# jgkellymit/GENIE-SMEM

Measured on AMD Instinct MI355X. Metric: query-bases/sec SMEM discovery, 100kb ref x 150bp reads; bit-exact SMEM set, higher is better.
Workload: dtype u8/int32 (2-bit packed bases, int32 SA rows; f64 only in the RMI predict)

## Files before the change

genie-smem_amd/csrc/kernels.hip:

```cpp
#include <hip/hip_runtime.h>

#include <algorithm>
#include <cstdio>
#include <cstdlib>
#include <mutex>
#include <string>
#include <unordered_map>

#include "genie_internal.h"

namespace genie {

namespace {

constexpr int kWave = 64;

__device__ __forceinline__ int rfl(int v) { return __builtin_amdgcn_readfirstlane(v); }
__device__ __forceinline__ void set_wave_priority(int i)
{
    switch (i & 3) {
    case 0: __builtin_amdgcn_s_setprio(0); break;
    case 1: __builtin_amdgcn_s_setprio(1); break;
    case 2: __builtin_amdgcn_s_setprio(2); break;
    default: __builtin_amdgcn_s_setprio(3); break;
// ... 446 lines not shown
#pragma unroll
    for (int off = 32; off > 0; off >>= 1) {
        const unsigned int lo = (unsigned)__shfl_xor((int)(unsigned)v, off, kWave);
        const unsigned int hi = (unsigned)__shfl_xor((int)(unsigned)(v >> 32), off, kWave);
        v += ((unsigned long long)hi << 32) | lo;
    }
    return v;
}

__device__ __forceinline__ unsigned long long wave_inclusive_scan64(unsigned long long v, int lane)
{
#pragma unroll
    for (int off = 1; off < kWave; off <<= 1) {
        const unsigned int lo = (unsigned)__shfl_up((int)(unsigned)v, off, kWave);
        const unsigned int hi = (unsigned)__shfl_up((int)(unsigned)(v >> 32), off, kWave);
        if (lane >= off) v += ((unsigned long long)hi << 32) | lo;
    }
    return v;
}

__global__ void __launch_bounds__(kScanBlock) compact_block_sums(const int32_t *__restrict__ counts, long long N, int cap,
                                                                 unsigned long long *__restrict__ block_sums)
{
    __shared__ unsigned long long wsum[kScanBlock / kWave];
    const long long i = (long long)blockIdx.x * kScanBlock + threadIdx.x;
    unsigned long long v = 0;
    if (i < N) { const int c = counts[i]; v = (unsigned long long)(c < 0 ? 0 : (c < cap ? c : cap)); }
    v = wave_sum64(v);
    if ((threadIdx.x & 63) == 0) wsum[threadIdx.x >> 6] = v;
    __syncthreads();
    if (threadIdx.x == 0) {
        unsigned long long s = 0;
        for (int w = 0; w < kScanBlock / kWave; w++) s += wsum[w];
        block_sums[blockIdx.x] = s;
    }
}

__global__ void __launch_bounds__(kScanBlock) scan_block_sums_kernel(unsigned long long *__restrict__ sums, long long nblocks)
{
    constexpr int kPer = 8;
    __shared__ unsigned long long wave_total[kScanBlock / kWave];
    __shared__ unsigned long long carry;
    const int lane = threadIdx.x & (kWave - 1), wave = threadIdx.x >> 6;
    if (threadIdx.x == 0) carry = 0;
    __syncthreads();
    for (long long base = 0; base < nblocks; base += (long long)kScanBlock * kPer) {
        const long long i0 = base + (long long)threadIdx.x * kPer;
        unsigned long long v[kPer], mine = 0;
#pragma unroll
        for (int e = 0; e < kPer; e++) {
            v[e] = i0 + e < nblocks ? sums[i0 + e] : 0ull;
            mine += v[e];
        }
        unsigned long long inc = mine;
#pragma unroll
        for (int off = 1; off < kWave; off <<= 1) {
            const unsigned int lo = (unsigned)__shfl_up((int)(unsigned)inc, off, kWave);
            const unsigned int hi = (unsigned)__shfl_up((int)(unsigned)(inc >> 32), off, kWave);
            if (lane >= off) inc += ((unsigned long long)hi << 32) | lo;
        }
        if (lane == kWave - 1) wave_total[wave] = inc;
        __syncthreads();
        unsigned long long before = carry, all = 0;
        for (int w = 0; w < kScanBlock / kWave; w++) {
            const unsigned long long t = wave_total[w];
            before += w < wave ? t : 0ull;
            all += t;
        }
        unsigned long long run = before + inc - mine;
#pragma unroll
        for (int e = 0; e < kPer; e++) {
            if (i0 + e < nblocks) sums[i0 + e] = run;
            run += v[e];
        }
        __syncthreads();
        if (threadIdx.x == 0) carry += all;
        __syncthreads();
    }
    if (threadIdx.x == 0) sums[nblocks] = carry;
}

__global__ void __launch_bounds__(kScanBlock) compact_scatter(const int32_t *__restrict__ counts,
                                                              const int4 *__restrict__ slots, long long N, int cap,
                                                              const unsigned long long *__restrict__ block_sums,
                                                              long long *__restrict__ offsets, int4 *__restrict__ out,
                                                              long long out_cap_rows)
{
    __shared__ unsigned long long wave_total[kScanBlock / kWave];
    const int lane = threadIdx.x & (kWave - 1), wave = threadIdx.x >> 6;
    const long long i = (long long)blockIdx.x * kScanBlock + threadIdx.x;
    unsigned long long v = 0;
    if (i < N) { const int c = counts[i]; v = (unsigned long long)(c < 0 ? 0 : (c < cap ? c : cap)); }
    const unsigned long long inc = wave_inclusive_scan64(v, lane);
    if (lane == kWave - 1) wave_total[wave] = inc;
    __syncthreads();
    unsigned long long base = block_sums[blockIdx.x] + inc - v;
    for (int w = 0; w < wave; w++) base += wave_total[w];
    if (i < N) {
        offsets[i] = (long long)base;
        if (i == N - 1) offsets[N] = (long long)(base + v);
        if (out) {
            const long long room = out_cap_rows - (long long)base;
            const unsigned int fit = room <= 0 ? 0u : (room < (long long)v ? (unsigned int)room : (unsigned int)v);
            for (unsigned int t = 0; t < fit; t++) out[base + t] = slots[i * (long long)cap + t];
        }
    }
}

std::mutex g_err_mu;
std::string g_err;

#define HIP_TRY(expr)                                                         \
    do {                                                                      \
        hipError_t e_ = (expr);                                               \
        if (e_ != hipSuccess) { set_hip_error(#expr, (int)e_); return GENIE_E_HIP; } \
    } while (0)

#define LAUNCH(kernel, grid, block, lds, stream, ...)                         \
    do {                                                                      \
        hipLaunchKernelGGL(kernel, grid, block, lds, stream, __VA_ARGS__);    \
        HIP_TRY(hipGetLastError());                                           \
    } while (0)

inline long long table_bytes(const genie_index *ix)
{
    return (long long)((ix->dev.flags & kFlagCompactTable) ? sizeof(MatchRec16) : sizeof(MatchRec)) * ix->dev.mtab_entries;
}

struct Geometry {
    int grid, block, lds;
    int grp;
    int wps;
    int wide;
    int max_len;
    int fwd_stride;
    int fwd_lds;
    int qp_recs;
    int qp_stride;
    int kj_row;
};

inline void shape_for(int max_len, Geometry *g)
{
    g->max_len = max_len;
    g->wide = max_len > 255;
    g->qp_recs = g->wide ? (max_len + 31) / 32 : ((max_len + 8 + 31) / 32 + 1 + 1) / 2;
    g->fwd_stride = g->wide ? ((max_len * 2) + 15) & ~15 : std::max(16, (max_len + 15) & ~15);
    int dw = std::max(1, (max_len + 3) / 4);
    if ((dw & 1) == 0) dw++;
    g->fwd_lds = dw * 4;
    g->kj_row = (std::max(max_len, 1) + 1 + 7) & ~7;
    g->qp_stride = g->wide ? g->qp_recs : g->qp_recs + kPairHeadWords * 8 / 16;
}

int plan_find_smems(const genie_index *ix, int mode, int max_len, long long N, Geometry *g)
{
    (void)mode;
    const int lds_cap = 160 * 1024;
    shape_for(max_len, g);
    const int cus = ix->num_cus > 0 ? ix->num_cus : 256;
    const int wpb = 8;
    long long per_block;
    if (g->wide) {
        g->grp = 1;
        g->lds = wpb * mt_long_wave_bytes(max_len, g->qp_recs) + 16;
        per_block = wpb;
    } else {
        const int ml = std::max(max_len, 1);
        const int grp = ix->opt_group_positions > 0 ? ix->opt_group_positions / ml : kMtTarget / ml;
        g->grp = std::max(1, std::min(std::min(kMtMaxG, kWave / mt_pack_dwords(ml) * 4), grp));
        g->lds = wpb * mt_wave_bytes(g->grp, ml, g->qp_recs, g->fwd_stride) + 16 + mt_quad_table_bytes(g->grp, ml);
        per_block = (long long)wpb * g->grp;
    }
    if (g->lds > lds_cap) return GENIE_E_TOO_LONG;
    g->block = wpb * kWave;
    g->wps = !g->wide && table_bytes(ix) > kTableFitsL2 ? 4 : ((ix->dev.flags & kFlagCompactTable) ? 6 : 8);
    int bpc = std::min(lds_cap / g->lds, 4 * g->wps / wpb);
    if (ix->opt_search_blocks_per_cu > 0) bpc = std::min(bpc, ix->opt_search_blocks_per_cu);
    if (bpc < 1) bpc = 1;
    long long gr = (long long)cus * bpc;
    const long long need = (N + per_block - 1) / per_block;
    if (gr > need) gr = need;
    if (gr < 1) gr = 1;
    g->grid = (int)gr;
    return GENIE_OK;
}

struct Workspace {
    uint8_t *fwd;
    RefRec *qp;
    int32_t *status;
    uint8_t *kj;
    int32_t *counts;
    uint8_t *scan_tmp;
    int32_t *vlens;
};

inline int64_t ws_align(int64_t x) { return (x + 255) & ~(int64_t)255; }

struct Carver {
    uint8_t *base;
    int64_t at = 0;
    template <class T> void take(T *&piece, int64_t bytes)
    {
        piece = base ? reinterpret_cast<T *>(base + at) : nullptr;
        at += ws_align(bytes);
    }
};

inline int64_t block_sums_bytes(int64_t N) { return (N / 16 + 3) * 8; }

inline int64_t workspace_layout(uint8_t *base, int64_t N, const Geometry &g, Workspace *ws, int64_t vlens_n = 0)
{
    Carver c{base};
    c.take(ws->fwd, N * (int64_t)g.fwd_stride);
    c.take(ws->qp, N * (int64_t)g.qp_stride * 16);
    c.take(ws->status, N * 4);
    c.take(ws->kj, N * (int64_t)g.kj_row * (g.wide ? 4 : 2));
    c.take(ws->counts, N * 4);
    c.take(ws->scan_tmp, block_sums_bytes(N));
    c.take(ws->vlens, vlens_n * 4);
    return c.at + 256;
}

inline int carve_workspace(void *d_ws, int64_t ws_bytes, int64_t N, const Geometry &g, Workspace *ws, int64_t vlens_n = 0)
{
    if (!d_ws || ws_bytes < workspace_layout(static_cast<uint8_t *>(d_ws), N, g, ws, vlens_n) || (reinterpret_cast<uintptr_t>(d_ws) & 255) != 0)
        return GENIE_E_CAPACITY;
    return GENIE_OK;
}

constexpr long long kLongTwoLaneReads = 32768;

struct FindRequest : FindBatch {
    int32_t *counts = nullptr, *slots = nullptr;
    int32_t cap = 0;
    int64_t *offsets = nullptr;
    int32_t *rows = nullptr;
    int64_t cap_rows = 0;
    bool packed = false;
    int row_bytes = 8;
    uint8_t *counts8 = nullptr, *status8 = nullptr;
    int64_t *escapes = nullptr;
    int64_t cap_escapes = 0;
    bool both = false;

    explicit FindRequest(const FindBatch &b) : FindBatch(b) {}
};

constexpr int kLdsBytes = 160 * 1024;
std::mutex g_lds_mu;
std::unordered_map<const void *, int> g_lds_limit;

template <class Kernel>
int allow_large_lds(Kernel k)
{
    const void *fn = reinterpret_cast<const void *>(k);
    int limit;
    {
        std::lock_guard<std::mutex> lk(g_lds_mu);
        auto it = g_lds_limit.find(fn);
        if (it == g_lds_limit.end()) {
            hipFuncAttributes attr;
            HIP_TRY(hipFuncGetAttributes(&attr, fn));
            it = g_lds_limit.emplace(fn, kLdsBytes - (int)attr.sharedSizeBytes).first;
        }
        limit = it->second;
    }
    HIP_TRY(hipFuncSetAttribute(fn, hipFuncAttributeMaxDynamicSharedMemorySize, limit));
    return GENIE_OK;
}

template <class Kernel, class... Args>
int launch_match_table(Kernel km, const Geometry &g, hipStream_t s, Args... args)
{
    if (int rc = allow_large_lds(km)) return rc;
    LAUNCH(km, dim3(g.grid), dim3(g.block), g.lds, s, args...);
    return GENIE_OK;
}

template <int MODE, bool WIDE>
int launch_pipeline(const genie_index *ix, const Geometry &g, const FindRequest &r, const Workspace &ws, hipStream_t s)
{
    int32_t *st = r.status ? r.status : ws.status;
    int32_t *cnt = r.counts ? r.counts : ws.counts;
    const bool c16 = (ix->dev.flags & kFlagCompactTable) != 0;
    const long long mtab_bytes = table_bytes(ix);
    const int cus = ix->num_cus > 0 ? ix->num_cus : 256;
    const int max_len = std::max(g.max_len, 1);
    const int long_flags = ix->opt_search_all | ix->opt_scheduling << 16, flags = long_flags | ix->opt_debug << 8;
    if (ix->ev_search_begin) HIP_TRY(hipEventRecord((hipEvent_t)ix->ev_search_begin, s));
    int rc;
    if (WIDE && r.both)
        rc = launch_match_table(c16 ? match_table_long_both_kernel<true> : match_table_long_both_kernel<false>, g, s, ix->dev,
                                (int)MODE, r.reads, r.lens, (long long)r.N, r.stride, r.fixed_len, reinterpret_cast<uint8_t *>(ws.fwd),
                                g.fwd_stride, ws.qp, g.qp_recs, st, max_len, mtab_bytes, long_flags, cus, ws.vlens);
    else if (WIDE)
        rc = launch_match_table(c16 ? match_table_long_kernel<true> : match_table_long_kernel<false>, g, s, ix->dev, (int)MODE,
                                r.reads, r.lens, (long long)r.N, r.stride, r.fixed_len, reinterpret_cast<uint8_t *>(ws.fwd),
                                g.fwd_stride, ws.qp, g.qp_recs, st, max_len, mtab_bytes, long_flags, cus);
    else if (r.both)
        rc = launch_match_table(c16 ? (g.wps == 4 ? match_table_both_kernel<4, true> : match_table_both_kernel<6, true>)
                                    : (g.wps == 4 ? match_table_both_kernel<4, false> : match_table_both_kernel<8, false>),
                                g, s, ix->dev, (int)MODE, r.reads, r.lens, (long long)r.N, r.stride, r.fixed_len,
                                reinterpret_cast<uint8_t *>(ws.fwd), g.fwd_stride, ws.qp, g.qp_recs, g.qp_stride, st, g.grp,
                                max_len, mtab_bytes, flags, cus, ws.vlens);
// ... 421 lines not shown
```

genie-smem_amd/csrc/match_table_body.inc:

```
    static_assert(!(PK && RC), "both strands of 2-bit packed reads are not built");
    typedef uint32_t __attribute__((aligned(1))) u32_unaligned;
    extern __shared__ __align__(16) uint8_t smem[];
    const int lane = threadIdx.x & (kWave - 1);
    const int wave = rfl((int)(threadIdx.x >> 6));
    const int waves_per_block = blockDim.x >> 6;
    const int dbg = (flags >> 8) & 63;
    const int sched = flags >> 16;
    const bool look_up_all = (flags & 1) != 0;
    const int FS = fwd_stride;
    const int K = ix.K;
    const int P2 = ix.P2;
    const int DW = mt_short_row_dwords(max_len, qp_recs);
    const int DWp = mt_pack_dwords(max_len);
    const int QL = mt_quads(max_len);
    const int nquads = grp * QL;
    const __amdgpu_buffer_rsrc_t mtab =
        __builtin_amdgcn_make_buffer_rsrc(const_cast<MatchRec *>(ix.mtab), 0, (int)mtab_bytes, 0x00020000);
    const __amdgpu_buffer_rsrc_t ov =
        __builtin_amdgcn_make_buffer_rsrc(const_cast<MatchOv16 *>(ix.ov), 0, ix.ov_entries * (int)sizeof(MatchOv16), 0x00020000);

    uint8_t *wb = smem + wave * mt_wave_bytes(grp, max_len, qp_recs, FS);
    uint32_t *Dp = reinterpret_cast<uint32_t *>(wb);
    int *Ls = reinterpret_cast<int *>(wb + mt_r16(grp * DW * 4));
    uint8_t *fwL = reinterpret_cast<uint8_t *>(Ls) + 64;
    uint16_t *sl = reinterpret_cast<uint16_t *>(fwL + mt_r16(grp * FS));
    uint16_t *qa = reinterpret_cast<uint16_t *>(reinterpret_cast<uint8_t *>(sl) + mt_r16(grp * max_len * 2));
    uint16_t *qb = qa + grp * mt_quads(max_len);
    for (int i = lane; i < grp * DW; i += kWave) Dp[i] = 0;
    const uint8_t *reads_end = reads + (RC ? N >> 1 : N) * (long long)stride;

    const int pu = (int)(((uint32_t)lane * (uint32_t)(65536 / DWp + 1)) >> 16);
    const int pj = lane - pu * DWp;

    uint32_t *next_group = reinterpret_cast<uint32_t *>(smem + waves_per_block * mt_wave_bytes(grp, max_len, qp_recs, FS));
    const long long groups = (N + grp - 1) / grp;
    const long long share = (groups + gridDim.x - 1) / gridDim.x;
    const long long g_begin = (long long)blockIdx.x * share;
    const long long g_end = g_begin + share < groups ? g_begin + share : groups;
    const bool handed_out = !(sched & 1), rotate = !(sched & 2);
    if (threadIdx.x == 0) *next_group = (uint32_t)waves_per_block;
    uint2 *qtab = reinterpret_cast<uint2 *>(next_group + 4);
    for (int t = threadIdx.x; t < (nquads + 191) / 192 * 192; t += blockDim.x) {
        const int tq = t < nquads ? t : 0;
        const int u = tq / QL, a = 4 * (tq - u * QL);
        const uint32_t o = 2u * (uint32_t)a + 1u;
        qtab[t] = make_uint2((uint32_t)u << 28 | (uint32_t)(u * FS + a) << 16 | (uint32_t)a,
                             ((uint32_t)(u * DW) + (o >> 5)) << 8 | (32u - (o & 31u)));
    }
    __syncthreads();
    long long gi = handed_out ? g_begin + wave : (long long)blockIdx.x * waves_per_block + wave;
    const long long g_stop = handed_out ? g_end : groups;
    const int round_of_block = (int)(blockIdx.x / (uint32_t)cus);
    const bool touch_ahead = !(sched & 8);
    for (int it = 0; gi < g_stop; it++) {
        const long long r = gi * grp;
        if (rotate) set_wave_priority(it + round_of_block);
        long long gi_next;
        if (handed_out) {
            uint32_t nx = 0;
            if (lane == 0) nx = atomicAdd(next_group, 1u);
            gi_next = g_begin + (long long)(uint32_t)rfl((int)nx);
        } else {
            gi_next = gi + (long long)gridDim.x * waves_per_block;
        }
        if (touch_ahead && stride > 0 && gi_next < g_stop) {
            const long long rn = gi_next * grp;
            const long long rows = N - rn < (long long)grp ? N - rn : (long long)grp;
            if (RC) scalar_touch_lines(reads + (rn >> 1) * (long long)stride, (uint32_t)((((rn + rows - 1) >> 1) - (rn >> 1) + 1) * stride));
            else scalar_touch_lines(reads + rn * (long long)stride, (uint32_t)(rows * stride));
        }
        bool any_read = false;
        for (int u0 = 0; u0 < grp; u0 += kWave / DWp) {
            const int u = u0 + pu;
            const bool mine = pu < kWave / DWp && u < grp;
            int L = 0, st = GENIE_READ_OK;
            uint32_t d = 0;
            bool bad = false;
            if (mine && r + u < N) {
                const long long row = RC ? (r + u) >> 1 : r + u;
                const bool rev = RC && ((r + u) & 1);
                L = lens ? lens[row] : fixed_len;
                if (RC && lens && pj == 0) vlens[r + u] = L;
                if (L < 0 || L > max_len) { st = GENIE_READ_BAD_BASE; L = 0; }
                const int left = L - 16 * pj;
                if (PK) {
                    if (left > 0) {
                        d = __builtin_bswap32(*reinterpret_cast<const uint32_t *>(reads + (r + u) * (long long)stride + 4 * pj));
                        if (left < 16) d &= ~0u << (32 - 2 * left);
                    }
                }
                const uint8_t *src = reads + row * (long long)stride + 16 * pj;
                uint32_t v[4] = {0, 0, 0, 0};
                if (PK) {
                } else if (rev) {
                    const long long o = row * (long long)stride + L - 16 - 16 * pj;
                    if (left >= 16 || (left > 0 && o >= 0)) {
                        const nt_u4 q = *reinterpret_cast<const nt_u4_unaligned *>(reads + o);
                        v[0] = __builtin_bswap32(q.w); v[1] = __builtin_bswap32(q.z); v[2] = __builtin_bswap32(q.y); v[3] = __builtin_bswap32(q.x);
                        if (left < 16) {
#pragma unroll
                            for (int k = 0; k < 4; k++) {
                                const int nb = left - 4 * k;
                                v[k] = nb >= 4 ? v[k] : (nb <= 0 ? 0u : v[k] & ((1u << (8 * nb)) - 1u));
                            }
                        }
                    } else if (left > 0) {
                        const uint8_t *f = reads + row * (long long)stride;
                        for (int b = 0; b < left; b++) v[b >> 2] |= (uint32_t)f[left - 1 - b] << (8 * (b & 3));
                    }
                } else if (left >= 16 || (left > 0 && src + 16 <= reads_end)) {
                    const nt_u4 q = *reinterpret_cast<const nt_u4_unaligned *>(src);
                    v[0] = q.x; v[1] = q.y; v[2] = q.z; v[3] = q.w;
                    if (left < 16) {
#pragma unroll
                        for (int k = 0; k < 4; k++) {
                            const int nb = left - 4 * k;
                            v[k] = nb >= 4 ? v[k] : (nb <= 0 ? 0u : v[k] & ((1u << (8 * nb)) - 1u));
                        }
                    }
                } else if (left > 0) {
#pragma unroll
                    for (int k = 0; k < 4; k++) {
                        if (left >= 4 * k + 4) v[k] = *reinterpret_cast<const u32_unaligned *>(src + 4 * k);
                        else for (int b = 0; b < left - 4 * k; b++) v[k] |= (uint32_t)src[4 * k + b] << (8 * b);
                    }
                }
                if (!PK) {
                    bad = ((v[0] | v[1] | v[2] | v[3]) & 0xFCFCFCFCu) != 0;
                    d = (mt_pack4(v[0]) << 24) | (mt_pack4(v[1]) << 16) | (mt_pack4(v[2]) << 8) | mt_pack4(v[3]);
                    if (rev && left > 0) d ^= left >= 16 ? ~0u : ~0u << (32 - 2 * left);
                }
            }
            const uint32_t prev = (uint32_t)__builtin_amdgcn_update_dpp(0, (int)d, 0x138 , 0xf, 0xf, true);
            const unsigned long long badm = __ballot(bad);
            bool ok = false;
            if (mine) {
                Dp[u * DW + pj] = __builtin_amdgcn_alignbit(prev, d, 1);
                if (pj == 0) {
                    const unsigned long long mine_bits = ((1ull << DWp) - 1ull) << (pu * DWp);
                    if (st == GENIE_READ_OK && (badm & mine_bits)) st = GENIE_READ_BAD_BASE;
                    if (st == GENIE_READ_OK && mode != GENIE_MODE_BWA && L < K) st = GENIE_READ_TOO_SHORT;
                    if (r + u < N) status[r + u] = st;
                    ok = st == GENIE_READ_OK && L > 0;
                    Ls[u] = ok ? L : 0;
                }
            }
            any_read |= __any(ok);
        }
        wave_lds_fence();
        if (any_read) {
            for (int t0 = 0; t0 < ((dbg & 8) ? 0 : grp * qp_recs); t0 += kWave) {
                const int t = t0 + lane;
                const int u = t / qp_recs, i = t - u * qp_recs;
                if (t < grp * qp_recs && Ls[u] > 0) {
                    const uint32_t *q = Dp + u * DW + 4 * i;
                    const uint32_t q0 = q[0], q1 = q[1], q2 = q[2], q3 = q[3], q4 = q[4];
                    uint4 rec;
                    rec.y = __builtin_amdgcn_alignbit(q0, q1, 31);
                    rec.x = __builtin_amdgcn_alignbit(q1, q2, 31);
                    rec.w = __builtin_amdgcn_alignbit(q2, q3, 31);
                    rec.z = __builtin_amdgcn_alignbit(q3, q4, 31);
                    store_nt(qp_out + (r + u) * (long long)qp_stride + i, rec);
                }
            }
            int nslow = 0;
#pragma nounroll
            for (int c0 = 0; c0 < ((dbg & 4) ? 0 : nquads); c0 += kMtNsp * kWave) {
                uint32_t ent[kMtNsp];
                MtProbe pr[kMtNsp];
#pragma unroll
                for (int s = 0; s < kMtNsp; s++) {
                    const int t0 = c0 + 64 * s + lane;
                    const uint2 q = qtab[t0];
                    int m = Ls[q.x >> 28] - (int)(q.x & 255u);
                    m = t0 < nquads && m > 0 ? m : 0;
                    ent[s] = q.x | ((uint32_t)m << 8);
                    const uint32_t *dq = Dp + (q.y >> 8);
                    const uint32_t sh = q.y & 255u;
                    const uint32_t d0 = dq[0], d1 = dq[1], d2 = dq[2];
                    pr[s] = mt_issue<C16>(mtab, __builtin_amdgcn_alignbit(d0, d1, sh), __builtin_amdgcn_alignbit(d1, d2, sh), P2);
                }
                mt_v4i rb[kMtNsp];
#pragma unroll
                for (int s = 0; s < kMtNsp; s++) rb[s] = mt_second<C16>(mtab, pr[s]);
#pragma unroll
                for (int s = 0; s < kMtNsp; s++) {
                    bool slow;
                    const int best0 = mt_eval<C16>(pr[s], rb[s], P2, slow);
                    const int a = (int)(ent[s] & 255u), m = (int)((ent[s] >> 8) & 255u);
                    const int best = best0 < m ? best0 : m;
                    if (m) fwL[(ent[s] >> 16) & 0xFFFu] = (uint8_t)(a + best);
                    slow = slow && m > best0;
                    const unsigned long long sb = __ballot(slow);
                    if (slow) sl[nslow + __popcll(sb & ((1ull << lane) - 1ull))] = (uint16_t)(((ent[s] >> 28) << 8) | (uint32_t)a);
                    nslow += __popcll(sb);
                }
            }
            wave_lds_fence();
#pragma nounroll
            for (int c0 = 0; c0 < ((dbg & 1) ? 0 : nslow); c0 += kWave) mt_slow<false, C16>(ix, mtab, ov, mode, lane, c0, nslow, sl, Dp, DW, Ls, fwL, FS);
            wave_lds_fence();
            nslow = 0;
            int nqa = 0, nqb = 0;
            const unsigned long long below = (1ull << lane) - 1ull;
#pragma nounroll
            for (int t0 = lane; t0 < ((dbg & 6) ? 0 : nquads) + lane; t0 += kWave) {
                const uint2 q = qtab[t0 < nquads ? t0 : 0];
                const int u = (int)(q.x >> 28), a = (int)(q.x & 255u);
                const int L = Ls[u];
                const int m = t0 < nquads && L > a ? L - a : 0;
                const uint32_t fo = (q.x >> 16) & 0xFFFu;
                const uint32_t v0 = fwL[fo];
                const bool has_right = m > 4;
                const uint32_t v4 = has_right ? fwL[fo + 4] : 0u;
                const bool need = m > 1 && (look_up_all || ((int)v0 != L && !(has_right && v4 == v0)));
                if (m && !need) *reinterpret_cast<uint32_t *>(fwL + fo) = v0 * 0x01010101u;
                const unsigned long long nb = __ballot(need);
                if (need) qa[nqa + __popcll(nb & below)] = (uint16_t)((uint32_t)u << 8 | (uint32_t)a);
                nqa += __popcll(nb);
            }
            wave_lds_fence();
#pragma nounroll
            for (int c0 = 0; c0 < nqa; c0 += kWave) {
                const bool valid = c0 + lane < nqa;
                const uint32_t it = qa[valid ? c0 + lane : 0];
                const int u = (int)(it >> 8), a = (int)(it & 255u);
                const int L = Ls[u], m = L - a;
                const int km = m > 2 ? 2 : 1;
                const uint32_t fo = __umul24((uint32_t)u, (uint32_t)FS) + (uint32_t)a;
                const uint32_t o = 2u * (uint32_t)(a + km) + 1u;
                const uint32_t *dq = Dp + __umul24((uint32_t)u, (uint32_t)DW) + (o >> 5);
                const uint32_t sh = 32u - (o & 31u);
                const uint32_t d0 = dq[0], d1 = dq[1], d2 = dq[2];
                const MtProbe pm = mt_issue<C16>(mtab, __builtin_amdgcn_alignbit(d0, d1, sh), __builtin_amdgcn_alignbit(d1, d2, sh), P2);
                const uint32_t v0 = fwL[fo];
                const bool has_right = m > 4;
                const uint32_t v4 = has_right ? fwL[fo + 4] : 0u;
                const mt_v4i rm = mt_second<C16>(mtab, pm);
                bool sm;
                const int bm = mt_eval<C16>(pm, rm, P2, sm);
                const int em = bm < m - km ? bm : m - km;
                sm = valid && sm && m - km > bm;
                const uint32_t vm = (uint32_t)(a + km + em);
                bool need1 = false, need3 = false;
                if (valid) {
                    if (km == 1) {
                        *reinterpret_cast<uint32_t *>(fwL + fo) = v0 | vm << 8;
                    } else {
                        need1 = look_up_all || sm || vm != v0;
                        need3 = m > 3 && (look_up_all || sm || !((has_right && vm == v4) || (int)vm == L));
                        *reinterpret_cast<uint32_t *>(fwL + fo) = v0 | v0 << 8 | vm << 16 | (m > 3 ? vm : 0u) << 24;
                    }
                }
                const unsigned long long sbm = __ballot(sm), b1 = __ballot(need1), b3 = __ballot(need3);
                if (sm) sl[nslow + __popcll(sbm & below)] = (uint16_t)(it + (uint32_t)km);
                nslow += __popcll(sbm);
                if (need1) qb[nqb + __popcll(b1 & below)] = (uint16_t)(it + 1u);
                nqb += __popcll(b1);
                if (need3) qb[nqb + __popcll(b3 & below)] = (uint16_t)(it + 3u);
                nqb += __popcll(b3);
            }
            wave_lds_fence();
#pragma nounroll
            for (int c0 = 0; c0 < nqb; c0 += kWave) {
                const bool valid = c0 + lane < nqb;
                const uint32_t it = qb[valid ? c0 + lane : 0];
                const int u = (int)(it >> 8), a = (int)(it & 255u);
                const int m = Ls[u] - a;
                const uint32_t o = 2u * (uint32_t)a + 1u;
                const uint32_t *dq = Dp + __umul24((uint32_t)u, (uint32_t)DW) + (o >> 5);
                const uint32_t sh = 32u - (o & 31u);
                const uint32_t d0 = dq[0], d1 = dq[1], d2 = dq[2];
                const MtProbe pn = mt_issue<C16>(mtab, __builtin_amdgcn_alignbit(d0, d1, sh), __builtin_amdgcn_alignbit(d1, d2, sh), P2);
                const mt_v4i rn = mt_second<C16>(mtab, pn);
                bool slow;
                const int b0 = mt_eval<C16>(pn, rn, P2, slow);
                const int e = b0 < m ? b0 : m;
                if (valid) fwL[__umul24((uint32_t)u, (uint32_t)FS) + (uint32_t)a] = (uint8_t)(a + e);
                slow = valid && slow && m > b0;
                const unsigned long long sb = __ballot(slow);
                if (slow) sl[nslow + __popcll(sb & below)] = (uint16_t)it;
                nslow += __popcll(sb);
            }
            wave_lds_fence();
#pragma nounroll
            for (int c0 = 0; c0 < ((dbg & 1) ? 0 : nslow); c0 += kWave) mt_slow<false, C16>(ix, mtab, ov, mode, lane, c0, nslow, sl, Dp, DW, Ls, fwL, FS);
            wave_lds_fence();
            const int nrows = N - r < (long long)grp ? (int)(N - r) : grp;
            uint4 *dst = reinterpret_cast<uint4 *>(fwd_out + r * (long long)FS);
            const uint4 *src = reinterpret_cast<const uint4 *>(fwL);
            for (int i = lane; i < ((dbg & 32) ? 0 : nrows * (FS >> 4)); i += kWave) store_nt(dst + i, src[i]);
        }
        wave_lds_fence();
        gi = gi_next;
    }
```

genie-smem_amd/csrc/match_table_kernel.inc:

```

constexpr int kMtNsp = 3;
constexpr int kMtMaxG = 16;
constexpr int kMtTarget = 768;


__host__ __device__ inline int mt_row_dwords(int max_len, int qp_recs)
{
    const int a = ((2 * (max_len + 8) + 1) >> 5) + 3, b = 2 * qp_recs + 3;
    return a > b ? a : b;
}
__host__ __device__ inline int mt_pack_dwords(int max_len) { return (max_len + 15) / 16 + 1; }
__host__ __device__ inline int mt_quads(int max_len) { return (max_len + 3) / 4; }
__host__ __device__ inline int mt_r16(int x) { return (x + 15) & ~15; }
__host__ __device__ inline int mt_quad_table_bytes(int grp, int max_len) { return (grp * mt_quads(max_len) + 191) / 192 * 192 * 8; }
__host__ __device__ inline int mt_short_row_dwords(int max_len, int chunks) { return mt_row_dwords(max_len, 2 * chunks - 1); }
__host__ __device__ inline int mt_wave_bytes(int grp, int max_len, int qp_recs, int fwd_stride)
{
    return mt_r16(grp * mt_short_row_dwords(max_len, qp_recs) * 4) + 64 + mt_r16(grp * fwd_stride) + mt_r16(grp * max_len * 2) +
           mt_r16(grp * mt_quads(max_len) * 6);
}

struct QBits {
    const uint32_t *p;
    __device__ __forceinline__ uint64_t win(int pos) const
    {
        const uint32_t o = 2u * (uint32_t)pos + 1u;
        const uint32_t *d = p + (o >> 5);
        const uint32_t s = 32u - (o & 31u);
        const uint32_t d0 = d[0], d1 = d[1], d2 = d[2];
        return ((uint64_t)__builtin_amdgcn_alignbit(d0, d1, s) << 32) | __builtin_amdgcn_alignbit(d1, d2, s);
    }
};

__device__ __forceinline__ uint32_t mt_pack4(uint32_t v) { return ((v << 6) | (v >> 4) | (v >> 14) | (v >> 24)) & 255u; }

struct MtProbe {
    uint32_t xk;
    int voff;
    mt_v4i ra;
};
template <bool C16>
__device__ __forceinline__ MtProbe mt_issue(const __amdgpu_buffer_rsrc_t mtab, uint32_t w1, uint32_t w2, int P2)
{
    MtProbe p;
    p.xk = __builtin_amdgcn_alignbit(w1, w2, 32 - 2 * P2);
    p.voff = (int)((w1 >> (32 - 2 * P2)) << (C16 ? 4 : 5));
    p.ra = __builtin_amdgcn_raw_buffer_load_b128(mtab, p.voff, 0, 0);
    return p;
}
template <bool C16>
__device__ __forceinline__ mt_v4i mt_second(const __amdgpu_buffer_rsrc_t mtab, const MtProbe &p)
{
    mt_v4i rb = mt_v4i{p.ra.z, p.ra.z, p.ra.z, p.ra.z};
    if (!C16 && ((uint32_t)p.ra.x >> 24) > 2u && p.xk > (uint32_t)p.ra.w) rb = __builtin_amdgcn_raw_buffer_load_b128(mtab, p.voff + 16, 0, 0);
    return rb;
}
typedef unsigned short mt_us2 __attribute__((ext_vector_type(2)));
__device__ __forceinline__ uint32_t mt_pk_min(uint32_t a, uint32_t b)
{
    return __builtin_bit_cast(uint32_t, __builtin_elementwise_min(__builtin_bit_cast(mt_us2, a), __builtin_bit_cast(mt_us2, b)));
}
__device__ __forceinline__ uint32_t mt_xmin16(const mt_v4i e, uint32_t xk16, bool more)
{
    const uint32_t xx = xk16 * 0x10001u;
    uint32_t d3 = (uint32_t)e.w ^ xx;
    d3 |= more ? 0xFFFF0000u : 0u;
    const uint32_t mm = mt_pk_min(mt_pk_min((uint32_t)e.y ^ xx, (uint32_t)e.z ^ xx), d3);
    return min(mm & 0xFFFFu, mm >> 16);
}
__device__ __forceinline__ int mt_lcp16(uint32_t x16) { return x16 ? (__clz((int)x16) - 16) >> 1 : 8; }
template <bool C16>
__device__ __forceinline__ int mt_eval(const MtProbe &p, const mt_v4i rb, int P2, bool &slow)
{
    if (C16) {
        const uint32_t w0 = (uint32_t)p.ra.x, cnt4 = (w0 >> 24) & 15u, nib = w0 >> 28;
        const bool wide = (nib & kM16Wide) && cnt4 >= 1u && cnt4 <= 3u;
        const bool rows_decide = cnt4 == kM16More || (cnt4 != 0 && !wide && (nib & kM16General));
        const uint32_t xx = wide ? p.xk : (p.xk >> 16) * 0x10001u;
        const uint32_t d1 = (uint32_t)p.ra.y ^ xx, d2 = (uint32_t)p.ra.z ^ xx, d3 = (uint32_t)p.ra.w ^ xx;
        const uint32_t mm = mt_pk_min(mt_pk_min(d1, d2), d3);
        const uint32_t xn = (min(mm & 0xFFFFu, mm >> 16) << 16) | 0xFFFFu;
        const uint32_t xw = min(min(d1, d2), d3);
        const int lcp = __clz((int)(wide ? xw : xn)) >> 1;
        slow = cnt4 != 0 && (rows_decide || lcp == (wide ? 16 : 8));
        return cnt4 == 0 ? (int)nib : (rows_decide ? P2 : P2 + lcp);
    }
    const uint32_t meta = (uint32_t)p.ra.x;
    uint32_t x = min(p.xk ^ (uint32_t)p.ra.z, p.xk ^ (uint32_t)p.ra.w);
    x = min(x, min(min(p.xk ^ (uint32_t)rb.x, p.xk ^ (uint32_t)rb.y), min(p.xk ^ (uint32_t)rb.z, p.xk ^ (uint32_t)rb.w)));
    const int lcp = __clz((int)x) >> 1;
    const int lm = (int)((meta >> 8) & 0x1Fu);
    slow = (meta & kMatchSlow) || lcp + lm == 16 + 0x1F;
    return (int)(meta & 0xFFu) + (lcp & lm);
}

struct MtQuad {
    uint32_t v1, v2, v3;
    bool s1, s2, s3;
};
template <bool C16>
__device__ __forceinline__ MtQuad mt_quad_interior(const __amdgpu_buffer_rsrc_t mtab, int P2, uint32_t d0, uint32_t d1, uint32_t d2,
                                                   uint32_t sh, int a, int m, int L, uint32_t v0, bool has_right, uint32_t v4,
                                                   bool look_up_all)
{
    MtQuad q{v0, 0u, 0u, false, false, false};
    const int km = m > 2 ? 2 : 1;
    const MtProbe pm = mt_issue<C16>(mtab, __builtin_amdgcn_alignbit(d0, d1, sh - 2 * km), __builtin_amdgcn_alignbit(d1, d2, sh - 2 * km), P2);
    const mt_v4i rm = mt_second<C16>(mtab, pm);
    bool sm;
    const int bm = mt_eval<C16>(pm, rm, P2, sm);
    const int em = bm < m - km ? bm : m - km;
    sm = sm && m - km > bm;
    const uint32_t vm = (uint32_t)(a + km + em);
    if (km == 1) {
        q.v1 = vm;
        q.s1 = sm;
        return q;
    }
    q.v2 = vm;
    q.s2 = sm;
    const bool need1 = look_up_all || sm || vm != v0;
    const bool need3 = m > 3 && (look_up_all || sm || !((has_right && vm == v4) || (int)vm == L));
    q.v1 = v0;
    q.v3 = m > 3 ? vm : 0u;
    if (need1 || need3) {
        const uint32_t s13 = need1 ? sh - 2 : sh - 6;
        const MtProbe pa = mt_issue<C16>(mtab, __builtin_amdgcn_alignbit(d0, d1, s13), __builtin_amdgcn_alignbit(d1, d2, s13), P2);
        MtProbe pb = pa;
        const bool both = need1 && need3;
        if (both) pb = mt_issue<C16>(mtab, __builtin_amdgcn_alignbit(d0, d1, sh - 6), __builtin_amdgcn_alignbit(d1, d2, sh - 6), P2);
        const mt_v4i ra = mt_second<C16>(mtab, pa);
        mt_v4i rb = ra;
        if (both) rb = mt_second<C16>(mtab, pb);
        bool sa, sb;
        const int ba = mt_eval<C16>(pa, ra, P2, sa), bb = mt_eval<C16>(pb, rb, P2, sb);
        const int ka = need1 ? 1 : 3;
        const int ea = ba < m - ka ? ba : m - ka, eb = bb < m - 3 ? bb : m - 3;
        sa = sa && m - ka > ba;
        sb = sb && m - 3 > bb;
        if (need1) { q.v1 = (uint32_t)(a + 1 + ea); q.s1 = sa; }
        else { q.v3 = (uint32_t)(a + 3 + ea); q.s3 = sa; }
        if (both) { q.v3 = (uint32_t)(a + 3 + eb); q.s3 = sb; }
    }
    return q;
}

template <bool LONG, bool C16, class QB = QBits, class FW = uint16_t>
__device__ __forceinline__ void mt_slow(const DevIndex &ix, const __amdgpu_buffer_rsrc_t mtab, const __amdgpu_buffer_rsrc_t ov, int mode, int lane, int c0,
                                        int count, const uint16_t *list, const uint32_t *Dp, int DW, const int *Ls,
                                        uint8_t *fwL, int FS, int L0 = 0, int wbase = 0, FW *fwW = nullptr)
{
    const int K = ix.K, P = ix.P, P2 = ix.P2;
    const int idx = c0 + lane;
    const bool on = idx < count;
    int u = 0, a = 0, m = 0, best = 0, chain = 0, cvoff = 0, nrows = 0;
    uint32_t mask = 0, lb = 0, c = 0, xmin = ~0u, xkq = 0;
    bool general = false;
    uint64_t w = 0, xq = 0;
    QB Q{reinterpret_cast<decltype(QB::p)>(Dp)};
    if (on) {
        const uint32_t e = (uint32_t)list[idx];
        if constexpr (LONG) {
            a = wbase + (int)e;
            m = L0 - a;
        } else {
            u = (int)(e >> 8);
            a = (int)(e & 255u);
            m = Ls[u] - a;
            Q.p = Dp + u * DW;
        }
        w = Q.win(a);
        xq = Q.win(a + P);
// ... 185 lines not shown
```

Baseline: 200.3 billion.

## Fuse quad-need scan into probe loop and defer plateau-dependent quads

The separate pass that re-read qtab and fwL to decide which quads need refinement is folded into the main probe loop, using per-quad slow-state bytes stored in a new LDS array. Quads whose outcome depends on an unresolved slow neighbour are placed on a deferred list and re-checked only after the slow path runs, so many skip the refinement probes. This removes one full LDS scan and a fence-separated slow pass before the scan, at the cost of extra LDS per wave, a second refinement trip, and more complex bookkeeping. A static_assert is added to keep three blocks per CU within LDS at 150 bases.

```diff
diff --git a/genie-smem_amd/csrc/kernels.hip b/genie-smem_amd/csrc/kernels.hip
--- a/genie-smem_amd/csrc/kernels.hip
+++ b/genie-smem_amd/csrc/kernels.hip
@@ -622,6 +622,9 @@
     g->kj_row = (std::max(max_len, 1) + 1 + 7) & ~7;
     g->qp_stride = g->wide ? g->qp_recs : g->qp_recs + kPairHeadWords * 8 / 16;
 }
+
+static_assert(3 * (8 * mt_wave_bytes(kMtTarget / 150, 150, 3, 160) + 16 + mt_quad_table_bytes(kMtTarget / 150, 150)) <= 160 * 1024,
+              "three blocks of the match-statistics kernel per CU no longer fit the LDS at 150 bases");
 
 int plan_find_smems(const genie_index *ix, int mode, int max_len, long long N, Geometry *g)
 {
diff --git a/genie-smem_amd/csrc/match_table_body.inc b/genie-smem_amd/csrc/match_table_body.inc
--- a/genie-smem_amd/csrc/match_table_body.inc
+++ b/genie-smem_amd/csrc/match_table_body.inc
@@ -26,6 +26,8 @@
     uint16_t *sl = reinterpret_cast<uint16_t *>(fwL + mt_r16(grp * FS));
     uint16_t *qa = reinterpret_cast<uint16_t *>(reinterpret_cast<uint8_t *>(sl) + mt_r16(grp * max_len * 2));
     uint16_t *qb = qa + grp * mt_quads(max_len);
+    uint16_t *qd = reinterpret_cast<uint16_t *>(reinterpret_cast<uint8_t *>(qa) + mt_r16(grp * mt_quads(max_len) * 6));
+    uint8_t *ss = reinterpret_cast<uint8_t *>(qd) + mt_r16(grp * mt_quads(max_len) * 2);
     for (int i = lane; i < grp * DW; i += kWave) Dp[i] = 0;
     const uint8_t *reads_end = reads + (RC ? N >> 1 : N) * (long long)stride;
 
@@ -163,7 +165,9 @@
                     store_nt(qp_out + (r + u) * (long long)qp_stride + i, rec);
                 }
             }
-            int nslow = 0;
+            int nslow = 0, nqa = 0, nqd = 0;
+            const unsigned long long below = (1ull << lane) - 1ull;
+            const bool list_on = !(dbg & 2);
 #pragma nounroll
             for (int c0 = 0; c0 < ((dbg & 4) ? 0 : nquads); c0 += kMtNsp * kWave) {
                 uint32_t ent[kMtNsp];
@@ -183,47 +187,60 @@
                 mt_v4i rb[kMtNsp];
 #pragma unroll
                 for (int s = 0; s < kMtNsp; s++) rb[s] = mt_second<C16>(mtab, pr[s]);
+                uint32_t vs[kMtNsp];
 #pragma unroll
                 for (int s = 0; s < kMtNsp; s++) {
                     bool slow;
                     const int best0 = mt_eval<C16>(pr[s], rb[s], P2, slow);
                     const int a = (int)(ent[s] & 255u), m = (int)((ent[s] >> 8) & 255u);
                     const int best = best0 < m ? best0 : m;
-                    if (m) fwL[(ent[s] >> 16) & 0xFFFu] = (uint8_t)(a + best);
                     slow = slow && m > best0;
+                    const bool plateau = C16 ? best0 != P2 : !((uint32_t)pr[s].ra.x & kMatchSlow);
+                    const uint32_t state = slow ? (plateau ? 2u : 1u) : 0u;
+                    vs[s] = (uint32_t)(a + best) | state << 8;
+                    if (m) {
+                        fwL[(ent[s] >> 16) & 0xFFFu] = (uint8_t)(a + best);
+                        ss[c0 + 64 * s + lane] = (uint8_t)state;
+                    }
                     const unsigned long long sb = __ballot(slow);
                     if (slow) sl[nslow + __popcll(sb & ((1ull << lane) - 1ull))] = (uint16_t)(((ent[s] >> 28) << 8) | (uint32_t)a);
                     nslow += __popcll(sb);
                 }
-            }
-            wave_lds_fence();
-#pragma nounroll
-            for (int c0 = 0; c0 < ((dbg & 1) ? 0 : nslow); c0 += kWave) mt_slow<false, C16>(ix, mtab, ov, mode, lane, c0, nslow, sl, Dp, DW, Ls, fwL, FS);
-            wave_lds_fence();
-            nslow = 0;
-            int nqa = 0, nqb = 0;
-            const unsigned long long below = (1ull << lane) - 1ull;
-#pragma nounroll
-            for (int t0 = lane; t0 < ((dbg & 6) ? 0 : nquads) + lane; t0 += kWave) {
-                const uint2 q = qtab[t0 < nquads ? t0 : 0];
-                const int u = (int)(q.x >> 28), a = (int)(q.x & 255u);
-                const int L = Ls[u];
-                const int m = t0 < nquads && L > a ? L - a : 0;
-                const uint32_t fo = (q.x >> 16) & 0xFFFu;
-                const uint32_t v0 = fwL[fo];
-                const bool has_right = m > 4;
-                const uint32_t v4 = has_right ? fwL[fo + 4] : 0u;
-                const bool need = m > 1 && (look_up_all || ((int)v0 != L && !(has_right && v4 == v0)));
-                if (m && !need) *reinterpret_cast<uint32_t *>(fwL + fo) = v0 * 0x01010101u;
-                const unsigned long long nb = __ballot(need);
-                if (need) qa[nqa + __popcll(nb & below)] = (uint16_t)((uint32_t)u << 8 | (uint32_t)a);
-                nqa += __popcll(nb);
-            }
-            wave_lds_fence();
+                wave_lds_fence();
+#pragma unroll
+                for (int s = 0; s < kMtNsp; s++) {
+                    const int a = (int)(ent[s] & 255u), m = (int)((ent[s] >> 8) & 255u);
+                    const int L = a + m;
+                    const uint32_t fo = (ent[s] >> 16) & 0xFFFu;
+                    const uint32_t v0 = vs[s] & 255u, s0 = vs[s] >> 8;
+                    const bool has_right = m > 4;
+                    const bool known = !(s == kMtNsp - 1 && lane == kWave - 1);
+                    const uint32_t v4 = has_right ? (known ? (uint32_t)fwL[fo + 4] : 256u) : 0u;
+                    const uint32_t s4 = has_right ? (known ? (uint32_t)ss[c0 + 64 * s + lane + 1] : 1u) : 0u;
+                    const bool x0 = s0 == 0u, x4 = s4 == 0u;
+                    const bool settled = x0 && ((int)v0 == L || (has_right && x4 && v4 == v0));
+                    const bool open = list_on && m > 1 && (look_up_all || !settled);
+                    const bool defer = open && !look_up_all && (x0 ? !x4 && v0 >= v4 : s0 == 2u);
+                    const bool need = open && !defer;
+                    if (list_on && m && !open) *reinterpret_cast<uint32_t *>(fwL + fo) = v0 * 0x01010101u;
+                    const unsigned long long nb = __ballot(need), db = __ballot(defer);
+                    const uint32_t item = (ent[s] >> 28) << 8 | (uint32_t)a;
+                    if (need) qa[nqa + __popcll(nb & below)] = (uint16_t)(item | (x0 ? 0u : 1u) | (x4 ? 0u : 2u));
+                    nqa += __popcll(nb);
+                    if (defer) qd[nqd + __popcll(db & below)] = (uint16_t)item;
+                    nqd += __popcll(db);
+                }
+            }
+            wave_lds_fence();
+            int nqb = 0;
+#pragma nounroll
+            for (int trip = 0;; trip++) {
 #pragma nounroll
             for (int c0 = 0; c0 < nqa; c0 += kWave) {
                 const bool valid = c0 + lane < nqa;
-                const uint32_t it = qa[valid ? c0 + lane : 0];
+                const uint32_t itf = qa[valid ? c0 + lane : 0];
+                const uint32_t it = itf & ~3u;
+                const bool f0 = (itf & 1u) != 0, f4 = (itf & 2u) != 0;
                 const int u = (int)(it >> 8), a = (int)(it & 255u);
                 const int L = Ls[u], m = L - a;
                 const int km = m > 2 ? 2 : 1;
@@ -247,8 +264,8 @@
                     if (km == 1) {
                         *reinterpret_cast<uint32_t *>(fwL + fo) = v0 | vm << 8;
                     } else {
-                        need1 = look_up_all || sm || vm != v0;
-                        need3 = m > 3 && (look_up_all || sm || !((has_right && vm == v4) || (int)vm == L));
+                        need1 = look_up_all || sm || f0 || vm != v0;
+                        need3 = m > 3 && (look_up_all || sm || !((has_right && !f4 && vm == v4) || (int)vm == L));
                         *reinterpret_cast<uint32_t *>(fwL + fo) = v0 | v0 << 8 | vm << 16 | (m > 3 ? vm : 0u) << 24;
                     }
                 }
@@ -286,6 +303,28 @@
 #pragma nounroll
             for (int c0 = 0; c0 < ((dbg & 1) ? 0 : nslow); c0 += kWave) mt_slow<false, C16>(ix, mtab, ov, mode, lane, c0, nslow, sl, Dp, DW, Ls, fwL, FS);
             wave_lds_fence();
+            if (trip || nqd == 0) break;
+            nqa = 0;
+#pragma nounroll
+            for (int c0 = 0; c0 < nqd; c0 += kWave) {
+                const bool valid = c0 + lane < nqd;
+                const uint32_t it = qd[valid ? c0 + lane : 0];
+                const int u = (int)(it >> 8), a = (int)(it & 255u);
+                const int L = Ls[u], m = L - a;
+                const uint32_t fo = __umul24((uint32_t)u, (uint32_t)FS) + (uint32_t)a;
+                const uint32_t v0 = fwL[fo];
+                const uint32_t v4 = m > 4 ? fwL[fo + 4] : ~0u;
+                const bool need = valid && (int)v0 != L && v4 != v0;
+                if (valid && !need) *reinterpret_cast<uint32_t *>(fwL + fo) = v0 * 0x01010101u;
+                const unsigned long long nb = __ballot(need);
+                if (need) qa[nqa + __popcll(nb & below)] = (uint16_t)it;
+                nqa += __popcll(nb);
+            }
+            wave_lds_fence();
+            if (nqa == 0) break;
+            nslow = 0;
+            nqb = 0;
+            }
             const int nrows = N - r < (long long)grp ? (int)(N - r) : grp;
             uint4 *dst = reinterpret_cast<uint4 *>(fwd_out + r * (long long)FS);
             const uint4 *src = reinterpret_cast<const uint4 *>(fwL);
diff --git a/genie-smem_amd/csrc/match_table_kernel.inc b/genie-smem_amd/csrc/match_table_kernel.inc
--- a/genie-smem_amd/csrc/match_table_kernel.inc
+++ b/genie-smem_amd/csrc/match_table_kernel.inc
@@ -4,20 +4,22 @@
 constexpr int kMtTarget = 768;
 
 
-__host__ __device__ inline int mt_row_dwords(int max_len, int qp_recs)
+__host__ __device__ constexpr int mt_row_dwords(int max_len, int qp_recs)
 {
     const int a = ((2 * (max_len + 8) + 1) >> 5) + 3, b = 2 * qp_recs + 3;
     return a > b ? a : b;
 }
-__host__ __device__ inline int mt_pack_dwords(int max_len) { return (max_len + 15) / 16 + 1; }
-__host__ __device__ inline int mt_quads(int max_len) { return (max_len + 3) / 4; }
-__host__ __device__ inline int mt_r16(int x) { return (x + 15) & ~15; }
-__host__ __device__ inline int mt_quad_table_bytes(int grp, int max_len) { return (grp * mt_quads(max_len) + 191) / 192 * 192 * 8; }
-__host__ __device__ inline int mt_short_row_dwords(int max_len, int chunks) { return mt_row_dwords(max_len, 2 * chunks - 1); }
-__host__ __device__ inline int mt_wave_bytes(int grp, int max_len, int qp_recs, int fwd_stride)
+__host__ __device__ constexpr int mt_pack_dwords(int max_len) { return (max_len + 15) / 16 + 1; }
+__host__ __device__ constexpr int mt_quads(int max_len) { return (max_len + 3) / 4; }
+__host__ __device__ constexpr int mt_r16(int x) { return (x + 15) & ~15; }
+__host__ __device__ constexpr int mt_quad_table_bytes(int grp, int max_len) { return (grp * mt_quads(max_len) + 191) / 192 * 192 * 8; }
+__host__ __device__ constexpr int mt_short_row_dwords(int max_len, int chunks) { return mt_row_dwords(max_len, 2 * chunks - 1); }
+__host__ __device__ constexpr int mt_wave_bytes(int grp, int max_len, int qp_recs, int fwd_stride)
 {
     return mt_r16(grp * mt_short_row_dwords(max_len, qp_recs) * 4) + 64 + mt_r16(grp * fwd_stride) + mt_r16(grp * max_len * 2) +
-           mt_r16(grp * mt_quads(max_len) * 6);
+           mt_r16(grp * mt_quads(max_len) * 6) +
+           mt_r16(grp * mt_quads(max_len) * 2) +
+           mt_r16(grp * mt_quads(max_len));
 }
 
 struct QBits {
```

Result: no change. 199.6 billion (-0.3%).
